# aubin-tchoi/shot-fpfh

Hardware: AMD Instinct MI355X
Metric: descriptors/sec (SHOT+FPFH) on 1M-pt cloud (higher is better)
Workload: dtype f64

## Files before the change

### shot_fpfh_amd/csrc/search.hip

```cpp
#include <algorithm>
#include <cmath>
#include <numeric>

#include "host_stage.h"
#include "search_util.h"

sf_grid_desc sf_make_grid_desc(const sf_cloud *c)
{
    sf_grid_desc g;
    for (int a = 0; a < 3; ++a) {
        g.lo[a] = c->lo[a];
        g.dim[a] = c->dim[a];
    }
    g.inv_cell = c->inv_cell;
    g.inv_cell_x = c->inv_cell * c->xsub;
    g.cell = c->cell;
    g.xsub = c->xsub;
    return g;
}

namespace {

__device__ unsigned long long sf_k2_paths[2];
template <int MODE, bool SEL, bool SHARE = false, bool DBG = false>
__global__ __launch_bounds__(64 * SF_K2_WPB) void k_radius(sf_grid_desc g, const int32_t *__restrict__ cell_start,
                                                const double *__restrict__ xs, const double *__restrict__ ys,
                                                const double *__restrict__ zs, const double *__restrict__ qx,
                                                const double *__restrict__ qy, const double *__restrict__ qz,
                                                int64_t m, double r2, int cap, int32_t *__restrict__ count,
                                                int64_t *__restrict__ offset, int32_t *__restrict__ idx,
                                                const int32_t *__restrict__ qsel)
{
    const int lane = threadIdx.x & 63, sl = lane & 15, rw = lane >> 4;
    const int64_t q0 = sf_uniform64((sf_xcd_block() * SF_K2_WPB + (threadIdx.x >> 6)) * 4);
    if (q0 >= m) return;
    const int nq = (int)(m - q0 < 4 ? m - q0 : 4);
    const int64_t qm0 = q0 + (rw < nq ? rw : 0);
    const int64_t qm = SEL ? (int64_t)qsel[qm0] : qm0;
    const double pxv = qx[qm], pyv = qy[qm], pzv = qz[qm];
    int y0, y1, z0, z1;
    stencil_bounds(pyv, g.lo[1], g.inv_cell, g.dim[1], y0, y1);
    stencil_bounds(pzv, g.lo[2], g.inv_cell, g.dim[2], z0, z1);
    __shared__ int4 runs[SF_K2_WPB][4][12];
    __shared__ int stages[MODE != 0 ? SF_K2_WPB : 1][SHARE ? 4 : 1][256];
    static_assert(!SHARE || (MODE == 2 && !SEL), "the shared sweep serves the single sweep into slots");
    int4(*const tabs)[12] = runs[threadIdx.x >> 6];
    bool share = false;
    int s, e;
    sf_k2_window(g, cell_start, pxv, pyv, pzv, r2, sl, rw < nq, y0, y1, z0, z1, s, e);
    if (SHARE) {
        const bool same = y0 == sf_uniform(y0) && y1 == sf_uniform(y1) && z0 == sf_uniform(z0) && z1 == sf_uniform(z1);
        share = nq == 4 && __ballot(same) == ~0ull;
        if (share) {
            int us = e > s ? s : 0x7fffffff, ue = e > s ? e : 0;
            us = min(us, __shfl_xor(us, 16));
            ue = max(ue, __shfl_xor(ue, 16));
            us = min(us, __shfl_xor(us, 32));
            ue = max(ue, __shfl_xor(ue, 32));
            s = ue ? us : 0;
            e = ue;
        }
    }
    const int first_slot = sf_k2_store_runs(s, e, sl, tabs[rw]);
    __builtin_amdgcn_wave_barrier();
    if (DBG && lane == 0) atomicAdd(&sf_k2_paths[share ? 0 : 1], 1ull);
    if (SHARE && share) {
        const int4 *const tab = tabs[0];
        const int b4 = __builtin_amdgcn_readlane(first_slot, 4), b8 = __builtin_amdgcn_readlane(first_slot, 8);
        const int nslots = __builtin_amdgcn_readlane(first_slot, 9);
        double px[4], py[4], pz[4];
        int total[4], flushed[4];
#pragma unroll
        for (int qi = 0; qi < 4; ++qi) {
            px[qi] = sf_read_lane(pxv, 16 * qi);
            py[qi] = sf_read_lane(pyv, 16 * qi);
            pz[qi] = sf_read_lane(pzv, 16 * qi);
            total[qi] = 0;
            flushed[qi] = 0;
        }
        int32_t *const out0 = idx + q0 * (int64_t)cap;
        for (int f0 = 0; f0 < nslots; f0 += 64) {
            const sf_k2_pair c = sf_k2_load_pair(tab, b4, b8, nslots, f0 + lane, xs, ys, zs);
            const int j = c.j;
            const unsigned long long i0 = __builtin_amdgcn_ballot_w64(c.in0), i1 = __builtin_amdgcn_ballot_w64(c.in1);
#pragma unroll
            for (int qi = 0; qi < 4; ++qi) {
                const double dxa = c.X.x - px[qi], dya = c.Y.x - py[qi], dza = c.Z.x - pz[qi];
                const double dxb = c.X.y - px[qi], dyb = c.Y.y - py[qi], dzb = c.Z.y - pz[qi];
                const double d2a = (dxa * dxa + dya * dya) + dza * dza, d2b = (dxb * dxb + dyb * dyb) + dzb * dzb;
                const bool hit0 = c.in0 & (d2a <= r2);
                const bool hit1 = c.in1 & (d2b <= r2);
                const unsigned long long m0 = __builtin_amdgcn_ballot_w64(d2a <= r2) & i0, m1 = __builtin_amdgcn_ballot_w64(d2b <= r2) & i1;
                int *const stage = stages[threadIdx.x >> 6][qi];
                const int2 pos = sf_k2_hit_pos(total[qi], m0, m1, hit0);
                if (hit0 && pos.x < cap) stage[pos.x & 255] = j;
                if (hit1 && pos.y < cap) stage[pos.y & 255] = j + 1;
                total[qi] += __popcll(m0) + __popcll(m1);
                const int have = total[qi] < cap ? total[qi] : cap;
                while (have - flushed[qi] >= 64) {
                    SF_LIST_STORE(out0 + qi * (int64_t)cap + flushed[qi] + lane, stage[(flushed[qi] + lane) & 255]);
                    flushed[qi] += 64;
                }
            }
        }
#pragma unroll
        for (int qi = 0; qi < 4; ++qi) {
            const int *const stage = stages[threadIdx.x >> 6][qi];
            const int have = total[qi] < cap ? total[qi] : cap;
            if (flushed[qi] + lane < have) SF_LIST_STORE(out0 + qi * (int64_t)cap + flushed[qi] + lane, stage[(flushed[qi] + lane) & 255]);
            if (lane == 0) {
                const int64_t q = q0 + qi;
                count[q] = total[qi];
                offset[q] = q * (int64_t)cap;
                if (q == m - 1) {
                    count[m] = 0;
                    offset[m] = (q + 1) * (int64_t)cap;
                }
            }
        }
        return;
    }
    for (int qi = 0; qi < nq; ++qi) {
        const int64_t q = SEL ? (int64_t)sf_uniform(__shfl((int)qm, 16 * qi)) : q0 + qi;
        const int4 *const tab = tabs[qi];
        const double px = __shfl(pxv, 16 * qi), py = __shfl(pyv, 16 * qi), pz = __shfl(pzv, 16 * qi);
        const int b4 = __shfl(first_slot, 16 * qi + 4), b8 = __shfl(first_slot, 16 * qi + 8);
#ifdef SF_K2_ABLATE
        const int nslots = sf_uniform(__shfl(first_slot, 16 * qi + 9)) * SF_K2_ABLATE / 100;
#else
        const int nslots = sf_uniform(__shfl(first_slot, 16 * qi + 9));
#endif
        int total = 0;
        const int64_t out = MODE == 1 ? offset[q] : q * (int64_t)cap;
        const int room = MODE == 2 ? cap : 0x7fffffff;
        int *const stage = stages[threadIdx.x >> 6][0];
        int flushed = 0;
        for (int f0 = 0; f0 < nslots; f0 += 64) {
            const sf_k2_pair c = sf_k2_load_pair(tab, b4, b8, nslots, f0 + lane, xs, ys, zs);
            const int j = c.j;
            const double dxa = c.X.x - px, dya = c.Y.x - py, dza = c.Z.x - pz;
            const double dxb = c.X.y - px, dyb = c.Y.y - py, dzb = c.Z.y - pz;
            const double d2a = (dxa * dxa + dya * dya) + dza * dza, d2b = (dxb * dxb + dyb * dyb) + dzb * dzb;
            const bool hit0 = c.in0 & (d2a <= r2);
            const bool hit1 = c.in1 & (d2b <= r2);
            const unsigned long long m0 = __ballot(hit0), m1 = __ballot(hit1);
            if (MODE != 0) {
                const int2 pos = sf_k2_hit_pos(total, m0, m1, hit0);
                if (hit0 && pos.x < room) stage[pos.x & 255] = j;
                if (hit1 && pos.y < room) stage[pos.y & 255] = j + 1;
            }
            total += __popcll(m0) + __popcll(m1);
            if (MODE != 0) {
                const int have = total < room ? total : room;
                while (have - flushed >= 64) {
                    SF_LIST_STORE(idx + out + flushed + lane, stage[(flushed + lane) & 255]);
                    flushed += 64;
                }
            }
        }
        if (MODE != 0) {
            const int have = total < room ? total : room;
            if (flushed + lane < have) SF_LIST_STORE(idx + out + flushed + lane, stage[(flushed + lane) & 255]);
        }
        if (lane == 0) {
            if (MODE != 1) {
                count[SEL ? q0 + qi : q] = total;
                if (!SEL && q == m - 1) count[m] = 0;
            }
            if (MODE == 2) {
                offset[q] = out;
                if (q == m - 1) offset[m] = out + cap;
            }
        }
    }
}

#ifndef SF_K2C_WPB
#define SF_K2C_WPB 4
#endif
#ifndef SF_K2C_LIST
#define SF_K2C_LIST 192
#endif
struct sf_cov_list { double x[SF_K2C_LIST], y[SF_K2C_LIST], z[SF_K2C_LIST]; };

__global__ __launch_bounds__(64 * SF_K2C_WPB) __attribute__((amdgpu_waves_per_eu(7))) void k_radius_cov(sf_grid_desc g, const int32_t *__restrict__ cell_start,
                                                const double *__restrict__ xs, const double *__restrict__ ys,
                                                const double *__restrict__ zs, const double *__restrict__ qx,
                                                const double *__restrict__ qy, const double *__restrict__ qz,
                                                int64_t m, double r2, double *__restrict__ cov, double *__restrict__ bary,
                                                int32_t *__restrict__ count)
{
    const int lane = threadIdx.x & 63, sl = lane & 15, rw = lane >> 4;
    const int64_t q0 = sf_uniform64((sf_xcd_block() * SF_K2C_WPB + (threadIdx.x >> 6)) * 4);
    if (q0 >= m) return;
    const int nq = (int)(m - q0 < 4 ? m - q0 : 4);
    const int64_t qm = q0 + (rw < nq ? rw : 0);
    const double pxv = qx[qm], pyv = qy[qm], pzv = qz[qm];
    int y0, y1, z0, z1;
    stencil_bounds(pyv, g.lo[1], g.inv_cell, g.dim[1], y0, y1);
    stencil_bounds(pzv, g.lo[2], g.inv_cell, g.dim[2], z0, z1);
    __shared__ int4 runs[SF_K2C_WPB][4][12];
    __shared__ sf_cov_list lists[SF_K2C_WPB];
    int4(*const tabs)[12] = runs[threadIdx.x >> 6];
    sf_cov_list &L = lists[threadIdx.x >> 6];
    int s, e;
    sf_k2_window(g, cell_start, pxv, pyv, pzv, r2, sl, rw < nq, y0, y1, z0, z1, s, e);
    const int first_slot = sf_k2_store_runs(s, e, sl, tabs[rw]);
    __builtin_amdgcn_wave_barrier();
#define SF_K2C_LDS_SYNC()                                                                                            \
    do {                                                                                                            \
        __builtin_amdgcn_fence(__ATOMIC_RELEASE, "wavefront");                                                      \
        __builtin_amdgcn_wave_barrier();                                                                            \
        __builtin_amdgcn_fence(__ATOMIC_ACQUIRE, "wavefront");                                                      \
    } while (0)
    for (int qi = 0; qi < nq; ++qi) {
        const int64_t q = q0 + qi;
        const int4 *const tab = tabs[qi];
        const double px = __shfl(pxv, 16 * qi), py = __shfl(pyv, 16 * qi), pz = __shfl(pzv, 16 * qi);
        const int b4 = __shfl(first_slot, 16 * qi + 4), b8 = __shfl(first_slot, 16 * qi + 8);
        const int nslots = sf_uniform(__shfl(first_slot, 16 * qi + 9));
        auto sweep = [&](int keep, bool wrap, auto &&after_step) -> int {
            int total = 0;
            for (int f0 = 0; f0 < nslots; f0 += 64) {
                const sf_k2_pair c = sf_k2_load_pair(tab, b4, b8, nslots, f0 + lane, xs, ys, zs);
                const double dxa = c.X.x - px, dya = c.Y.x - py, dza = c.Z.x - pz;
                const double dxb = c.X.y - px, dyb = c.Y.y - py, dzb = c.Z.y - pz;
                const double d2a = (dxa * dxa + dya * dya) + dza * dza, d2b = (dxb * dxb + dyb * dyb) + dzb * dzb;
                const bool hit0 = c.in0 & (d2a <= r2);
                const bool hit1 = c.in1 & (d2b <= r2);
                const unsigned long long m0 = __ballot(hit0), m1 = __ballot(hit1);
                const int2 pos = sf_k2_hit_pos(total, m0, m1, hit0);
                const int s0 = wrap ? pos.x % SF_K2C_LIST : pos.x, s1 = wrap ? pos.y % SF_K2C_LIST : pos.y;
                if (hit0 && pos.x < keep) { L.x[s0] = dxa; L.y[s0] = dya; L.z[s0] = dza; }
                if (hit1 && pos.y < keep) { L.x[s1] = dxb; L.y[s1] = dyb; L.z[s1] = dzb; }
                total += __popcll(m0) + __popcll(m1);
                after_step(total);
            }
            return total;
        };
        SF_K2C_LDS_SYNC();
        const int k = sweep(SF_K2C_LIST, false, [](int) {});
        SF_K2C_LDS_SYNC();
        const double kk = (double)k, ik = 1.0 / kk;
        double sx = 0.0, sy = 0.0, sz = 0.0;
        double part[8] = {0, 0, 0, 0, 0, 0, 0, 0};
        double mx, my, mz;
        if (k <= SF_K2C_LIST) {
            for (int t = lane; t < k; t += 64) { sx += L.x[t]; sy += L.y[t]; sz += L.z[t]; }
            {
                const double bs[4] = {sx, sy, sz, 0.0};
                const double bt = sf_wave_sum4(bs);
                mx = sf_read_lane(bt, 0) * ik; my = sf_read_lane(bt, 16) * ik; mz = sf_read_lane(bt, 32) * ik;
            }
            for (int t = lane; t < k; t += 64) {
                const double ax = L.x[t] - mx, ay = L.y[t] - my, az = L.z[t] - mz;
                part[0] += ax * ax;
                part[1] += ay * ax;
                part[2] += az * ax;
                part[3] += ay * ay;
                part[4] += az * ay;
                part[5] += az * az;
            }
        } else {
            int done = 0;
            auto bary_step = [&](int total) {
                if (done + 64 <= total) {
                    SF_K2C_LDS_SYNC();
                    while (done + 64 <= total) {
                        const int t = (done + lane) % SF_K2C_LIST;
                        sx += L.x[t]; sy += L.y[t]; sz += L.z[t];
                        done += 64;
                    }
                    SF_K2C_LDS_SYNC();
                }
            };
            sweep(0x7fffffff, true, bary_step);
            SF_K2C_LDS_SYNC();
            if (done + lane < k) { const int t = (done + lane) % SF_K2C_LIST; sx += L.x[t]; sy += L.y[t]; sz += L.z[t]; }
            {
                const double bs[4] = {sx, sy, sz, 0.0};
                const double bt = sf_wave_sum4(bs);
                mx = sf_read_lane(bt, 0) * ik; my = sf_read_lane(bt, 16) * ik; mz = sf_read_lane(bt, 32) * ik;
            }
            auto add_moments = [&](int t) {
                const double ax = L.x[t] - mx, ay = L.y[t] - my, az = L.z[t] - mz;
                part[0] += ax * ax;
                part[1] += ay * ax;
                part[2] += az * ax;
                part[3] += ay * ay;
                part[4] += az * ay;
                part[5] += az * az;
            };
            done = 0;
            auto mom_step = [&](int total) {
                if (done + 64 <= total) {
                    SF_K2C_LDS_SYNC();
                    while (done + 64 <= total) {
                        add_moments((done + lane) % SF_K2C_LIST);
                        done += 64;
                    }
                    SF_K2C_LDS_SYNC();
                }
            };
            SF_K2C_LDS_SYNC();
            sweep(0x7fffffff, true, mom_step);
            SF_K2C_LDS_SYNC();
            if (done + lane < k) add_moments((done + lane) % SF_K2C_LIST);
        }
        const double tot = sf_wave_sum8(part);
        const int e = lane >> 3;
        if ((lane & 7) == 0 && e < 6) cov[6 * q + e] = tot * ik;
        if (bary && lane == 0) { bary[3 * q] = mx; bary[3 * q + 1] = my; bary[3 * q + 2] = mz; }
        if (count && lane == 0) count[q] = k;
    }
#undef SF_K2C_LDS_SYNC
}

__global__ void k_query_cells(const double *__restrict__ q, int64_t m, sf_grid_desc g, int32_t *__restrict__ cid,
                              int32_t *__restrict__ val)
{
    int64_t i = (int64_t)blockIdx.x * blockDim.x + threadIdx.x;
    if (i >= m) return;
    int cx = sf_cell_coord(q[3 * i + 0], g.lo[0], g.inv_cell_x, g.dim[0]);
    int cy = sf_cell_coord(q[3 * i + 1], g.lo[1], g.inv_cell, g.dim[1]);
    int cz = sf_cell_coord(q[3 * i + 2], g.lo[2], g.inv_cell, g.dim[2]);
    cid[i] = (cz * g.dim[1] + cy) * g.dim[0] + cx;
    val[i] = (int32_t)i;
// ... 187 lines not shown
    }
    nb->planned = true;
    nb->main_chunks = chunks;
    nb->n_mid = 0;
    for (int c = chunks; c < 4; ++c) nb->n_mid += nb->hist[c];
    if (chunks == need) nb->n_mid = 0;
    nb->tail_limit = 255;
    nb->n_tail = nb->hist[4];
    if (nb->max_count <= nb->tail_limit) { nb->tail_limit = 0x7fffffff; nb->n_tail = 0; }
    if (nb->n_mid) SF_CHECK(select_slots(ctx, m, count_between{nb->count, 64 * chunks, 255}, nb->n_mid, &nb->mid_sel));
    if (nb->n_tail) SF_CHECK(select_longer(ctx, nb->count, m, nb->tail_limit, nb->n_tail, &nb->tail_sel));
    return SF_OK;
}

static int64_t capacity_from(const sf_cloud *c, double mean, int64_t mx)
{
    int64_t v = (int64_t)(std::max(mean * 2.25, 1.15 * (double)mx)) + 32;
    return std::min<int64_t>(((v + 31) / 32) * 32, std::max<int64_t>(((c->n + 31) / 32) * 32, 32));
}

static int sample_capacity(sf_ctx *ctx, sf_cloud *c, sf_nbrs *nb, const sf_grid_desc &g, double r2, int64_t *cap)
{
    const int64_t m = nb->m, stride = m / SF_K2_SAMPLE;
    sf_pool_guard tmp(ctx);
    int32_t *sel = nullptr, *cnt = nullptr;
    void *pin = nullptr;
    SF_CHECK(tmp.alloc(&sel, (size_t)SF_K2_SAMPLE));
    SF_CHECK(tmp.alloc(&cnt, (size_t)SF_K2_SAMPLE));
    SF_CHECK(sf_ctx_pinned(ctx, &pin));
    static_assert(SF_K2_SAMPLE * sizeof(int32_t) <= SF_PINNED_BYTES, "sample exceeds the pinned words");
    SF_LAUNCH(ctx, "k2_sample", k_iota_stride, dim3(SF_K2_SAMPLE / 256), dim3(256), sel, (int64_t)SF_K2_SAMPLE, stride);
    SF_LAUNCH(ctx, "k2_sample", (k_radius<0, true>), dim3(sf_xcd_grid(sf_div_up(SF_K2_SAMPLE, 4 * SF_K2_WPB))), dim3(64 * SF_K2_WPB), g,
              c->cell_start, c->xs, c->ys, c->zs, nb->qx, nb->qy, nb->qz, (int64_t)SF_K2_SAMPLE, r2, 0, cnt, (int64_t *)nullptr,
              (int32_t *)nullptr, (const int32_t *)sel);
    SF_HIP(hipMemcpyAsync(pin, cnt, SF_K2_SAMPLE * sizeof(int32_t), hipMemcpyDeviceToHost, ctx->stream));
    SF_HIP(hipStreamSynchronize(ctx->stream));
    const int32_t *h = (const int32_t *)pin;
    double sum = 0.0;
    int32_t mx = 0;
    for (int i = 0; i < SF_K2_SAMPLE; ++i) { sum += h[i]; mx = std::max(mx, h[i]); }
    *cap = capacity_from(c, sum / SF_K2_SAMPLE, mx);
    return SF_OK;
}

int sf_k2_count_sample(sf_ctx *ctx, sf_cloud *c, sf_nbrs *nb, double r2, int32_t *sel_dev, int32_t *cnt_dev)
{
    const sf_grid_desc g = sf_make_grid_desc(c);
    sf_launch_timer t_(ctx, "k2_sample");
    hipLaunchKernelGGL(k_iota_stride, dim3(SF_K2_SAMPLE / 256), dim3(256), 0, ctx->stream, sel_dev, (int64_t)SF_K2_SAMPLE, nb->m / SF_K2_SAMPLE);
    hipLaunchKernelGGL((k_radius<0, true>), dim3(sf_xcd_grid(sf_div_up(SF_K2_SAMPLE, 4 * SF_K2_WPB))), dim3(64 * SF_K2_WPB), 0, ctx->stream, g,
                       c->cell_start, c->xs, c->ys, c->zs, nb->qx, nb->qy, nb->qz, (int64_t)SF_K2_SAMPLE, r2, 0, cnt_dev, (int64_t *)nullptr,
                       (int32_t *)nullptr, (const int32_t *)sel_dev);
    SF_HIP(hipGetLastError());
    return SF_OK;
}

static int exact_scan_fill(sf_ctx *ctx, sf_cloud *c, sf_nbrs *nb, const sf_grid_desc &g, const dim3 &grid, const dim3 &block, double r2)
{
    const int64_t m = nb->m;
    {
        sf_pool_guard tmp(ctx);
        auto in = rocprim::make_transform_iterator(nb->count, to_i64());
        SF_CHECK(sf_rocprim(ctx, tmp, "k2_scan", true, [&](void *t, size_t &tb) {
            return rocprim::exclusive_scan(t, tb, in, nb->offset, (int64_t)0, (size_t)(m + 1), rocprim::plus<int64_t>(), ctx->stream);
        }));
    }
    SF_CHECK(sf_palloc(ctx, &nb->idx, (size_t)nb->total + 4));
    nb->cap = 0;
    if (nb->total) {
        SF_LAUNCH(ctx, "k2_radius_fill", (k_radius<1, false>), grid, block, g, c->cell_start, c->xs, c->ys, c->zs, nb->qx, nb->qy,
                  nb->qz, m, r2, 0, nb->count, nb->offset, nb->idx, (const int32_t *)nullptr);
    }
    return SF_OK;
}

static int run_search(sf_ctx *ctx, sf_cloud *c, sf_nbrs *nb)
{
    const int64_t m = nb->m;
    const double r2 = nb->radius * nb->radius;
    SF_CHECK(sf_palloc(ctx, &nb->count, (size_t)(m + 1)));
    SF_CHECK(sf_palloc(ctx, &nb->offset, (size_t)(m + 1)));
    if (!m) {
        SF_HIP(hipMemsetAsync(nb->count, 0, sizeof(int32_t), ctx->stream));
        SF_HIP(hipMemsetAsync(nb->offset, 0, sizeof(int64_t), ctx->stream));
    }
    sf_grid_desc g = sf_make_grid_desc(c);
    const dim3 grid(sf_xcd_grid(sf_div_up(m ? m : 1, 4 * SF_K2_WPB))), block(64 * SF_K2_WPB);
    if (!m) {
        if (ctx->collective_stats && ctx->comm) {
            const sf_cloud::search_key ekey{nb->radius, c->cell, c->xsub, nb->self_begin, 0};
            const bool seen = nb->self && !getenv("SF_K2_NO_HINT") && c->search_records.count(ekey);
            if (!seen || getenv("SF_K2_CHECK_RECORD")) {
                SF_CHECK(count_stats(ctx, nb, 0x7fffffff, nullptr));
                if (nb->self) {
                    sf_cloud::search_record r;
                    r.max_count_all = (int32_t)nb->max_count_all;
                    r.folded = true;
                    c->search_records[ekey] = r;
                }
            } else {
                nb->max_count_all = c->search_records[ekey].max_count_all;
            }
        }
        SF_CHECK(sf_palloc(ctx, &nb->idx, (size_t)8));
        return SF_OK;
    }
    int64_t cap = 0;
    bool optimistic = m >= 8 * SF_K2_SAMPLE && !getenv("SF_K2_EXACT");
    if (optimistic) {
        auto hint = c->list_stats.find({nb->radius, nb->self});
        if (hint != c->list_stats.end() && !getenv("SF_K2_NO_HINT")) cap = capacity_from(c, hint->second.first, hint->second.second);
        else SF_CHECK(sample_capacity(ctx, c, nb, g, r2, &cap));
        if (const char *e = getenv("SF_K2_CAP")) { const long v = atol(e); if (v >= 32) cap = (v / 32) * 32; }
        const int64_t most = std::max<int64_t>(((((int64_t)24 << 30) / (4 * m)) / 32) * 32, 32);
        if (cap > most) cap = std::max<int64_t>(most, 64);
        optimistic = cap * m * 4 <= ((int64_t)24 << 30) && cap < 0x7fffffff;
    }
    if (!optimistic) {
        SF_LAUNCH(ctx, "k2_radius_count", (k_radius<0, false>), grid, block, g, c->cell_start, c->xs, c->ys, c->zs, nb->qx, nb->qy,
                  nb->qz, m, r2, 0, nb->count, nb->offset, (int32_t *)nullptr, (const int32_t *)nullptr);
        const sf_cloud::search_key xkey{nb->radius, c->cell, c->xsub, nb->self_begin, -m};
        auto xit = nb->self && !getenv("SF_K2_NO_HINT") && !getenv("SF_K2_CHECK_RECORD") ? c->search_records.find(xkey) : c->search_records.end();
        if (xit != c->search_records.end() && (xit->second.folded || !(ctx->collective_stats && ctx->comm))) {
            const sf_cloud::search_record &r = xit->second;
            nb->total = r.total;
            nb->max_count = r.max_count;
            nb->max_count_all = r.max_count_all;
            nb->n_overflow = 0;
            for (int h = 0; h < 5; ++h) nb->hist[h] = r.hist[h];
        } else {
            SF_CHECK(count_stats(ctx, nb, 0x7fffffff, nullptr));
            if (nb->self) {
                if (c->search_records.size() > 256) c->search_records.clear();
                sf_cloud::search_record r;
                r.total = nb->total; r.max_count = nb->max_count; r.max_count_all = nb->max_count_all;
                for (int h = 0; h < 5; ++h) r.hist[h] = nb->hist[h];
                r.folded = ctx->collective_stats && ctx->comm;
                c->search_records[xkey] = r;
            }
        }
        SF_CHECK(exact_scan_fill(ctx, c, nb, g, grid, block, r2));
        return plan_dispatch(ctx, c, nb);
    }
    const sf_cloud::search_key rkey{nb->radius, c->cell, c->xsub, nb->self_begin, m};
    const sf_cloud::search_record *rec = nullptr;
    if (nb->self && !getenv("SF_K2_NO_HINT")) {
        auto it = c->search_records.find(rkey);
        if (it != c->search_records.end() && (it->second.folded || !(ctx->collective_stats && ctx->comm))) rec = &it->second;
    }
    if (rec) cap = rec->cap;
    SF_CHECK(sf_palloc(ctx, &nb->idx, (size_t)(cap * m) + 4));
    nb->cap = cap;
    const char *const sh = getenv("SF_K2_SHARED");
    const int shared = sh ? atoi(sh) : 1;
    auto *const k_slots = shared == 2 ? k_radius<2, false, true, true> : shared ? k_radius<2, false, true> : k_radius<2, false>;
    SF_LAUNCH(ctx, "k2_radius_slots", k_slots, grid, block, g, c->cell_start, c->xs, c->ys, c->zs, nb->qx, nb->qy,
              nb->qz, m, r2, (int)cap, nb->count, nb->offset, nb->idx, (const int32_t *)nullptr);
    int64_t ovf_total = 0;
    if (rec && !getenv("SF_K2_CHECK_RECORD")) {
        nb->total = rec->total;
        nb->max_count = rec->max_count;
        nb->max_count_all = rec->max_count_all;
        nb->n_overflow = rec->n_overflow;
        for (int h = 0; h < 5; ++h) nb->hist[h] = rec->hist[h];
        ovf_total = rec->ovf_total;
    } else {
        SF_CHECK(count_stats(ctx, nb, (int)cap, &ovf_total));
        if (rec && (nb->total != rec->total || nb->max_count != rec->max_count || nb->n_overflow != rec->n_overflow ||
                    ovf_total != rec->ovf_total || nb->hist[4] != rec->hist[4] || nb->hist[0] != rec->hist[0])) {
            sf_set_error("sf_radius_search_self: the lists of positions %lld .. + %lld at radius %g differ from the record of the previous "
                         "search of that range (total %lld / %lld)", (long long)nb->self_begin, (long long)m, nb->radius,
                         (long long)nb->total, (long long)rec->total);
            return SF_ERR_STATE;
        }
        if (nb->self) {
            if (c->search_records.size() > 256) c->search_records.clear();
            sf_cloud::search_record r;
            r.total = nb->total; r.n_overflow = nb->n_overflow; r.ovf_total = ovf_total; r.cap = cap;
            for (int h = 0; h < 5; ++h) r.hist[h] = nb->hist[h];
            r.max_count = nb->max_count; r.max_count_all = nb->max_count_all;
            r.folded = ctx->collective_stats && ctx->comm;
            if (r.n_overflow) {
                const int64_t most = std::max<int64_t>(((((int64_t)24 << 30) / (4 * m)) / 32) * 32, 32);
                const int64_t cap2 = capacity_from(c, (double)nb->total / (double)m, nb->max_count);
                if (cap2 >= nb->max_count && cap2 <= most) { r.cap = cap2; r.n_overflow = 0; r.ovf_total = 0; }
            }
            c->search_records[rkey] = r;
        }
    }
    if (nb->n_overflow * 2 > m) {
        sf_pool_release(ctx, nb->idx);
        nb->idx = nullptr;
        nb->n_overflow = 0;
        SF_CHECK(exact_scan_fill(ctx, c, nb, g, grid, block, r2));
        return plan_dispatch(ctx, c, nb);
    }
    if (nb->n_overflow) {
        const int64_t no = nb->n_overflow;
        sf_pool_guard tmp(ctx);
        int32_t *sel = nullptr;
        int64_t *off = nullptr;
        SF_CHECK(select_longer(ctx, nb->count, m, (int)cap, no, &sel));
        tmp.held.push_back(sel);
        SF_CHECK(tmp.alloc(&off, (size_t)no));
        auto in = rocprim::make_transform_iterator((const int32_t *)sel, count_of{nb->count});
        SF_CHECK(sf_rocprim(ctx, tmp, "k2_scan", true, [&](void *t, size_t &tb) {
            return rocprim::exclusive_scan(t, tb, in, off, (int64_t)0, (size_t)no, rocprim::plus<int64_t>(), ctx->stream);
        }));
        SF_CHECK(sf_palloc(ctx, &nb->idx_ovf, (size_t)ovf_total + 4));
        const int64_t delta = (int64_t)(((intptr_t)nb->idx_ovf - (intptr_t)nb->idx) / (intptr_t)sizeof(int32_t));
        SF_LAUNCH(ctx, "k2_select", k_patch_offsets, dim3((unsigned)sf_div_up(no, 256)), dim3(256), (const int32_t *)sel,
                  (const int64_t *)off, no, delta, nb->offset);
        SF_LAUNCH(ctx, "k2_radius_refill", (k_radius<1, true>), dim3(sf_xcd_grid(sf_div_up(no, 4 * SF_K2_WPB))), block, g, c->cell_start,
                  c->xs, c->ys, c->zs, nb->qx, nb->qy, nb->qz, no, r2, 0, nb->count, nb->offset, nb->idx, (const int32_t *)sel);
    }
    return plan_dispatch(ctx, c, nb);
}

static int ensure_grid(sf_ctx *ctx, sf_cloud *c, double radius, int64_t need_begin = 0, int64_t need_end = -1)
{
    if (!(radius > 0.0) || !std::isfinite(radius)) {
        sf_set_error("radius must be positive and finite (got %g)", radius);
        return SF_ERR_ARG;
    }
    const bool covers = need_end < 0 ? (c->pop_begin == 0 && c->pop_end == c->n)
                                     : (need_begin >= c->pop_begin && need_end <= c->pop_end);
    if (c->cell_start && covers && c->cell >= radius && c->cell <= 2.0 * radius * (1.0 + 1e-6)) return SF_OK;
    return sf_cloud_build_grid(ctx, c, radius);
}

extern "C" sf_nbrs *sf_radius_search_self(sf_ctx *ctx, sf_cloud *c, double radius, int64_t begin, int64_t end)
{
    if (!ctx || !c) { sf_set_error("sf_radius_search_self: null argument"); return nullptr; }
    if (begin < 0 || end > c->n || begin > end) {
        sf_set_error("sf_radius_search_self: bad range [%lld, %lld) for n=%lld", (long long)begin, (long long)end,
                     (long long)c->n);
        return nullptr;
    }
    if (hipSetDevice(ctx->device) != hipSuccess) { sf_set_error("hipSetDevice failed"); return nullptr; }
    if (ensure_grid(ctx, c, radius, begin, end) != SF_OK) return nullptr;
    sf_nbrs *nb = new sf_nbrs();
    nb->m = end - begin;
    nb->radius = radius;
    nb->self = true;
    nb->self_begin = begin;
    nb->qx = c->xs + begin;
    nb->qy = c->ys + begin;
    nb->qz = c->zs + begin;
    sf_nbrs_stamp(nb, c);
    if (run_search(ctx, c, nb) != SF_OK) {
        sf_nbrs_free(ctx, nb);
        return nullptr;
    }
    return nb;
}

int sf_k2_prepare_queries(sf_ctx *ctx, sf_cloud *c, sf_nbrs *nb, const double *queries, int flags)
{
    const int64_t m = nb->m;
    size_t mm = (size_t)(m ? m : 1);
    double *dq = nullptr;
    bool own_dq = false;
    if (flags & SF_IN_DEVICE) {
        dq = const_cast<double *>(queries);
    } else {
        SF_CHECK(sf_palloc(ctx, &dq, mm * 3));
        own_dq = true;
        if (m) SF_HIP(hipMemcpyAsync(dq, queries, (size_t)m * 24, hipMemcpyHostToDevice, ctx->stream));
    }
    SF_CHECK(sf_palloc(ctx, &nb->qx, mm));
    SF_CHECK(sf_palloc(ctx, &nb->qy, mm));
    SF_CHECK(sf_palloc(ctx, &nb->qz, mm));
    SF_CHECK(sf_palloc(ctx, &nb->qrow, mm));
    if (m) {
        sf_pool_guard tmp(ctx);
        int32_t *cid = nullptr, *cid_s = nullptr, *val = nullptr;
        SF_CHECK(tmp.alloc(&cid, mm));
        SF_CHECK(tmp.alloc(&cid_s, mm));
        SF_CHECK(tmp.alloc(&val, mm));
        sf_grid_desc g = sf_make_grid_desc(c);
        SF_LAUNCH(ctx, "k2_query_cells", k_query_cells, dim3((unsigned)sf_div_up(m, 256)), dim3(256), dq, m, g, cid,
                  val);
        int bits = 1;
        while (((int64_t)1 << bits) < c->ncell) ++bits;
        SF_CHECK(sf_rocprim(ctx, tmp, "k2_query_sort", true, [&](void *t, size_t &tb) {
            return rocprim::radix_sort_pairs<sf_sort_config>(t, tb, cid, cid_s, val, nb->qrow, (size_t)m, 0, bits, ctx->stream);
        }));
        SF_LAUNCH(ctx, "k2_gather_queries", k_gather_queries, dim3((unsigned)sf_div_up(m, 256)), dim3(256), dq,
                  nb->qrow, m, nb->qx, nb->qy, nb->qz);
    }
    if (own_dq) {
        SF_HIP(hipStreamSynchronize(ctx->stream));
        sf_pool_release(ctx, dq);
    }
    return SF_OK;
}

extern "C" sf_nbrs *sf_radius_search(sf_ctx *ctx, sf_cloud *c, const double *queries, int64_t m, double radius,
                                     int flags)
{
    if (!ctx || !c || (!queries && m > 0) || m < 0 || m > 2147483000LL) {
        sf_set_error("sf_radius_search: bad arguments (m=%lld)", (long long)m);
        return nullptr;
    }
    if (hipSetDevice(ctx->device) != hipSuccess) { sf_set_error("hipSetDevice failed"); return nullptr; }
    if (ensure_grid(ctx, c, radius) != SF_OK) return nullptr;
    sf_nbrs *nb = new sf_nbrs();
    nb->m = m;
    nb->radius = radius;
    nb->self = false;
// ... 362 lines not shown
```

### shot_fpfh_amd/csrc/search_util.h

```cpp
#pragma once
#include "common.h"
#include "dev_prims.h"
#include "device_util.h"

namespace {


struct to_i64 {
    __host__ __device__ int64_t operator()(int32_t v) const { return (int64_t)v; }
};

__device__ inline void stencil_bounds(double v, double lo, double inv_cell, int dim, int &c0, int &c1)
{
    double t = floor((v - lo) * inv_cell);
    double top = (double)(dim - 1);
    double a = t - 1.0, b = t + 1.0;
    if (!(a >= 0.0)) a = 0.0;
    if (a > top) a = top;
    if (!(b >= 0.0)) b = 0.0;
    if (b > top) b = top;
    c0 = (int)a;
    c1 = (int)b;
}


#ifndef SF_K2_WPB
#define SF_K2_WPB 8
#endif

__device__ __forceinline__ void sf_k2_window(const sf_grid_desc &g, const int32_t *__restrict__ cell_start, double px, double py,
                                             double pz, double r2, int sl, bool row_live, int y0, int y1, int z0, int z1, int &s,
                                             int &e)
{
    const int r = sl < 9 ? sl : 8;
    const int cz = z0 + r / 3, cy = y0 + r % 3;
    bool ok = sl < 9 && row_live && cz <= z1 && cy <= y1;
    const int64_t row = ((int64_t)(ok ? cz : z0) * g.dim[1] + (ok ? cy : y0)) * g.dim[0];
    const double pxr = px - g.lo[0], pyr = py - g.lo[1], pzr = pz - g.lo[2];
    const double by0 = (double)cy * g.cell, bz0 = (double)cz * g.cell;
    const double slack_y = 1e-9 * g.cell + 1e-15 * (fabs(pyr) + by0 + g.cell);
    const double slack_z = 1e-9 * g.cell + 1e-15 * (fabs(pzr) + bz0 + g.cell);
    const double dy = fmax(fmax(by0 - pyr, pyr - (by0 + g.cell)) - slack_y, 0.0);
    const double dz = fmax(fmax(bz0 - pzr, pzr - (bz0 + g.cell)) - slack_z, 0.0);
    const double w2 = (r2 * (1.0 + 1e-9) - dy * dy) - dz * dz;
    ok = ok && w2 >= 0.0;
    const double w = sf_sqrt_fast(fmax(w2, 0.0)) * (1.0 + 1e-9) + 1e-9 * g.cell +
                     1e-15 * (fabs(pxr) + (double)g.dim[0] * (g.cell / (double)g.xsub));
    s = 0;
    e = 0;
    if (sl < 9) {
        s = cell_start[row + sf_cell_coord(pxr - w, 0.0, g.inv_cell_x, g.dim[0])];
        e = cell_start[row + sf_cell_coord(pxr + w, 0.0, g.inv_cell_x, g.dim[0]) + 1];
    }
    if (!ok) { s = 0; e = 0; }
}

__device__ __forceinline__ int sf_k2_store_runs(int s, int e, int sl, int4 *tab_row)
{
    const int base = s & ~1;
    const int npairs = (e - base + 1) >> 1;
    int inc = npairs;
    inc += __builtin_amdgcn_update_dpp(0, inc, 0x111, 0xf, 0xf, false);
    inc += __builtin_amdgcn_update_dpp(0, inc, 0x112, 0xf, 0xf, false);
    inc += __builtin_amdgcn_update_dpp(0, inc, 0x114, 0xf, 0xf, false);
    inc += __builtin_amdgcn_update_dpp(0, inc, 0x118, 0xf, 0xf, false);
    const int first_slot = inc - npairs;
    if (sl < 12) tab_row[sl] = make_int4(base - 2 * first_slot, s, e, first_slot);
    return first_slot;
}

struct sf_k2_pair {
    int j;
    bool in0, in1;
    double2 X, Y, Z;
};
__device__ __forceinline__ sf_k2_pair sf_k2_load_pair(const int4 *tab, int b4, int b8, int nslots, int f, const double *__restrict__ xs,
                                                      const double *__restrict__ ys, const double *__restrict__ zs)
{
    int r = f >= b4 ? 4 : 0;
    r += f >= tab[r + 2].w ? 2 : 0;
    r += f >= tab[r + 1].w ? 1 : 0;
    r = f >= b8 ? 8 : r;
    const int4 t = tab[r];
    const bool live = f < nslots;
    sf_k2_pair p;
    p.j = live ? t.x + 2 * f : 0;
    p.in0 = live & (p.j >= t.y);
    p.in1 = live & (p.j + 1 < t.z);
    p.X = *reinterpret_cast<const double2 *>(xs + p.j);
    p.Y = *reinterpret_cast<const double2 *>(ys + p.j);
    p.Z = *reinterpret_cast<const double2 *>(zs + p.j);
    return p;
}

__device__ __forceinline__ int2 sf_k2_hit_pos(int total, unsigned long long m0, unsigned long long m1, bool hit0)
{
    const int pos = total + sf_prefix_count(m0) + sf_prefix_count(m1);
    return make_int2(pos, pos + (hit0 ? 1 : 0));
}

#define SF_K2_SAMPLE 2048

struct sf_identity {
    template <typename T> __host__ __device__ T operator()(T v) const { return v; }
};
template <typename S, typename T, typename F>
__global__ void k_perm_scatter(const S *__restrict__ sorted, const int32_t *__restrict__ perm, int64_t n, T *__restrict__ out, F f)
{
    const int64_t i = (int64_t)blockIdx.x * blockDim.x + threadIdx.x;
    if (i < n) out[perm[i]] = f(sorted[i]);
}
template <typename T>
__global__ void k_perm_gather(const T *__restrict__ src, const int32_t *__restrict__ perm, int64_t n, int pad, T *__restrict__ sorted)
{
    const int64_t i = (int64_t)blockIdx.x * blockDim.x + threadIdx.x;
    if (i < n) sorted[i] = src[perm[i]];
    else if (i < n + pad) sorted[i] = T(0);
}
template <typename S, typename T, typename F = sf_identity>
int sf_perm_scatter(sf_ctx *ctx, const char *name, const sf_cloud *c, const S *sorted, T *out, F f = F())
{
    SF_LAUNCH(ctx, name, (k_perm_scatter<S, T, F>), dim3((unsigned)sf_div_up(c->n, 256)), dim3(256), sorted, (const int32_t *)c->perm, c->n, out, f);
    return SF_OK;
}
template <typename T>
int sf_perm_gather(sf_ctx *ctx, const char *name, const sf_cloud *c, const T *src, int pad, T *sorted)
{
    SF_LAUNCH(ctx, name, k_perm_gather<T>, dim3((unsigned)sf_div_up(c->n + pad, 256)), dim3(256), src, (const int32_t *)c->perm, c->n, pad, sorted);
    return SF_OK;
}

}

int sf_k2_prepare_queries(sf_ctx *ctx, sf_cloud *c, sf_nbrs *nb, const double *queries, int flags);
int sf_k2_count_sample(sf_ctx *ctx, sf_cloud *c, sf_nbrs *nb, double r2, int32_t *sel_dev, int32_t *cnt_dev);
int sf_k2_ensure_grid(sf_ctx *ctx, sf_cloud *c, double radius);
int sf_k2_own_grid(sf_ctx *ctx, sf_cloud *c, double radius);
int sf_k2_radius_cov_self(sf_ctx *ctx, sf_cloud *c, double radius, const char *prof, double *cov, int32_t *count);
int sf_k2_count_self(sf_ctx *ctx, sf_cloud *c, double radius, const char *prof, int32_t *count);
int sf_k2_ball_sizes(sf_ctx *ctx, sf_cloud *c, sf_pool_guard &g, double radius, const char *prof, int32_t **count);
```

Baseline: 611.6 million.

## Share candidate sweep across eight queries per wave in radius search

Adds a new radius-search kernel in which each wave handles eight queries instead of four. When all eight share the same y/z stencil, it builds a single union candidate window and tests every loaded candidate pair against all eight query points read from LDS. This amortizes candidate loads and the window and run-table setup over more queries. It also uses a 128-entry ring per query with spill handling, and a single-point tail that handles leftover slots at half-pair granularity. The new kernel is the default; in exchange it uses more LDS per block, adds per-hit bookkeeping, and scans a wider union window when the eight queries' x ranges differ.

```diff
diff --git a/shot_fpfh_amd/csrc/search.hip b/shot_fpfh_amd/csrc/search.hip
--- a/shot_fpfh_amd/csrc/search.hip
+++ b/shot_fpfh_amd/csrc/search.hip
@@ -22,18 +22,17 @@
 namespace {
 
 __device__ unsigned long long sf_k2_paths[2];
-template <int MODE, bool SEL, bool SHARE = false, bool DBG = false>
-__global__ __launch_bounds__(64 * SF_K2_WPB) void k_radius(sf_grid_desc g, const int32_t *__restrict__ cell_start,
-                                                const double *__restrict__ xs, const double *__restrict__ ys,
-                                                const double *__restrict__ zs, const double *__restrict__ qx,
-                                                const double *__restrict__ qy, const double *__restrict__ qz,
-                                                int64_t m, double r2, int cap, int32_t *__restrict__ count,
-                                                int64_t *__restrict__ offset, int32_t *__restrict__ idx,
-                                                const int32_t *__restrict__ qsel)
+template <int MODE, bool SEL, bool SHARE, bool DBG, bool QLDS = false>
+__device__ __forceinline__ void sf_k2_four(const sf_grid_desc &g, const int32_t *__restrict__ cell_start,
+                                           const double *__restrict__ xs, const double *__restrict__ ys,
+                                           const double *__restrict__ zs, const double *__restrict__ qx,
+                                           const double *__restrict__ qy, const double *__restrict__ qz,
+                                           int64_t m, double r2, int cap, int32_t *__restrict__ count,
+                                           int64_t *__restrict__ offset, int32_t *__restrict__ idx,
+                                           const int32_t *__restrict__ qsel, const int64_t q0, int4 (*const tabs)[12],
+                                           int (*const stages)[256], double *const qc = nullptr)
 {
     const int lane = threadIdx.x & 63, sl = lane & 15, rw = lane >> 4;
-    const int64_t q0 = sf_uniform64((sf_xcd_block() * SF_K2_WPB + (threadIdx.x >> 6)) * 4);
-    if (q0 >= m) return;
     const int nq = (int)(m - q0 < 4 ? m - q0 : 4);
     const int64_t qm0 = q0 + (rw < nq ? rw : 0);
     const int64_t qm = SEL ? (int64_t)qsel[qm0] : qm0;
@@ -41,10 +40,7 @@
     int y0, y1, z0, z1;
     stencil_bounds(pyv, g.lo[1], g.inv_cell, g.dim[1], y0, y1);
     stencil_bounds(pzv, g.lo[2], g.inv_cell, g.dim[2], z0, z1);
-    __shared__ int4 runs[SF_K2_WPB][4][12];
-    __shared__ int stages[MODE != 0 ? SF_K2_WPB : 1][SHARE ? 4 : 1][256];
     static_assert(!SHARE || (MODE == 2 && !SEL), "the shared sweep serves the single sweep into slots");
-    int4(*const tabs)[12] = runs[threadIdx.x >> 6];
     bool share = false;
     int s, e;
     sf_k2_window(g, cell_start, pxv, pyv, pzv, r2, sl, rw < nq, y0, y1, z0, z1, s, e);
@@ -70,11 +66,15 @@
         const int nslots = __builtin_amdgcn_readlane(first_slot, 9);
         double px[4], py[4], pz[4];
         int total[4], flushed[4];
+        if (QLDS) {
+            if (sl == 0) { qc[rw] = pxv; qc[8 + rw] = pyv; qc[16 + rw] = pzv; }
+            __builtin_amdgcn_wave_barrier();
+        }
 #pragma unroll
         for (int qi = 0; qi < 4; ++qi) {
-            px[qi] = sf_read_lane(pxv, 16 * qi);
-            py[qi] = sf_read_lane(pyv, 16 * qi);
-            pz[qi] = sf_read_lane(pzv, 16 * qi);
+            px[qi] = QLDS ? 0.0 : sf_read_lane(pxv, 16 * qi);
+            py[qi] = QLDS ? 0.0 : sf_read_lane(pyv, 16 * qi);
+            pz[qi] = QLDS ? 0.0 : sf_read_lane(pzv, 16 * qi);
             total[qi] = 0;
             flushed[qi] = 0;
         }
@@ -83,15 +83,18 @@
             const sf_k2_pair c = sf_k2_load_pair(tab, b4, b8, nslots, f0 + lane, xs, ys, zs);
             const int j = c.j;
             const unsigned long long i0 = __builtin_amdgcn_ballot_w64(c.in0), i1 = __builtin_amdgcn_ballot_w64(c.in1);
+            int step0 = 0;
+            if (QLDS) asm volatile("" : "+v"(step0));
 #pragma unroll
             for (int qi = 0; qi < 4; ++qi) {
-                const double dxa = c.X.x - px[qi], dya = c.Y.x - py[qi], dza = c.Z.x - pz[qi];
-                const double dxb = c.X.y - px[qi], dyb = c.Y.y - py[qi], dzb = c.Z.y - pz[qi];
+                const double qpx = QLDS ? qc[step0 + qi] : px[qi], qpy = QLDS ? qc[step0 + 8 + qi] : py[qi], qpz = QLDS ? qc[step0 + 16 + qi] : pz[qi];
+                const double dxa = c.X.x - qpx, dya = c.Y.x - qpy, dza = c.Z.x - qpz;
+                const double dxb = c.X.y - qpx, dyb = c.Y.y - qpy, dzb = c.Z.y - qpz;
                 const double d2a = (dxa * dxa + dya * dya) + dza * dza, d2b = (dxb * dxb + dyb * dyb) + dzb * dzb;
                 const bool hit0 = c.in0 & (d2a <= r2);
                 const bool hit1 = c.in1 & (d2b <= r2);
                 const unsigned long long m0 = __builtin_amdgcn_ballot_w64(d2a <= r2) & i0, m1 = __builtin_amdgcn_ballot_w64(d2b <= r2) & i1;
-                int *const stage = stages[threadIdx.x >> 6][qi];
+                int *const stage = stages[qi];
                 const int2 pos = sf_k2_hit_pos(total[qi], m0, m1, hit0);
                 if (hit0 && pos.x < cap) stage[pos.x & 255] = j;
                 if (hit1 && pos.y < cap) stage[pos.y & 255] = j + 1;
@@ -105,7 +108,7 @@
         }
 #pragma unroll
         for (int qi = 0; qi < 4; ++qi) {
-            const int *const stage = stages[threadIdx.x >> 6][qi];
+            const int *const stage = stages[qi];
             const int have = total[qi] < cap ? total[qi] : cap;
             if (flushed[qi] + lane < have) SF_LIST_STORE(out0 + qi * (int64_t)cap + flushed[qi] + lane, stage[(flushed[qi] + lane) & 255]);
             if (lane == 0) {
@@ -133,7 +136,7 @@
         int total = 0;
         const int64_t out = MODE == 1 ? offset[q] : q * (int64_t)cap;
         const int room = MODE == 2 ? cap : 0x7fffffff;
-        int *const stage = stages[threadIdx.x >> 6][0];
+        int *const stage = stages[0];
         int flushed = 0;
         for (int f0 = 0; f0 < nslots; f0 += 64) {
             const sf_k2_pair c = sf_k2_load_pair(tab, b4, b8, nslots, f0 + lane, xs, ys, zs);
@@ -173,6 +176,163 @@
             }
         }
     }
+}
+
+template <int MODE, bool SEL, bool SHARE = false, bool DBG = false>
+__global__ __launch_bounds__(64 * SF_K2_WPB) void k_radius(sf_grid_desc g, const int32_t *__restrict__ cell_start,
+                                                const double *__restrict__ xs, const double *__restrict__ ys,
+                                                const double *__restrict__ zs, const double *__restrict__ qx,
+                                                const double *__restrict__ qy, const double *__restrict__ qz,
+                                                int64_t m, double r2, int cap, int32_t *__restrict__ count,
+                                                int64_t *__restrict__ offset, int32_t *__restrict__ idx,
+                                                const int32_t *__restrict__ qsel)
+{
+    const int64_t q0 = sf_uniform64((sf_xcd_block() * SF_K2_WPB + (threadIdx.x >> 6)) * 4);
+    if (q0 >= m) return;
+    __shared__ int4 runs[SF_K2_WPB][4][12];
+    __shared__ int stages[MODE != 0 ? SF_K2_WPB : 1][SHARE ? 4 : 1][256];
+    sf_k2_four<MODE, SEL, SHARE, DBG>(g, cell_start, xs, ys, zs, qx, qy, qz, m, r2, cap, count, offset, idx, qsel, q0,
+                                      runs[threadIdx.x >> 6], stages[MODE != 0 ? threadIdx.x >> 6 : 0]);
+}
+
+#ifndef SF_K2_WPB8
+#define SF_K2_WPB8 8
+#endif
+#define SF_K2_RING8 128
+template <bool DBG>
+__global__ __launch_bounds__(64 * SF_K2_WPB8) __attribute__((amdgpu_waves_per_eu(6))) void k_radius8(sf_grid_desc g, const int32_t *__restrict__ cell_start,
+                                                const double *__restrict__ xs, const double *__restrict__ ys,
+                                                const double *__restrict__ zs, const double *__restrict__ qx,
+                                                const double *__restrict__ qy, const double *__restrict__ qz,
+                                                int64_t m, double r2, int cap, int32_t *__restrict__ count,
+                                                int64_t *__restrict__ offset, int32_t *__restrict__ idx)
+{
+    const int lane = threadIdx.x & 63, sl = lane & 15, rw = lane >> 4, wv = threadIdx.x >> 6;
+    const int64_t q0 = sf_uniform64((sf_xcd_block() * SF_K2_WPB8 + wv) * 8);
+    if (q0 >= m) return;
+    __shared__ int4 runs[SF_K2_WPB8][4][12];
+    __shared__ double qcs[SF_K2_WPB8][3][8];
+    __shared__ int stages[SF_K2_WPB8][8 * SF_K2_RING8];
+    static_assert(8 * SF_K2_RING8 == 4 * 256, "the two halves' four-query sweeps run in the same LDS");
+    int4(*const tabs)[12] = runs[wv];
+    if (m - q0 >= 8) {
+        const double pxa = qx[q0 + rw], pya = qy[q0 + rw], pza = qz[q0 + rw];
+        const double pxb = qx[q0 + rw + 4], pyb = qy[q0 + rw + 4], pzb = qz[q0 + rw + 4];
+        int y0, y1, z0, z1, yb0, yb1, zb0, zb1;
+        stencil_bounds(pya, g.lo[1], g.inv_cell, g.dim[1], y0, y1);
+        stencil_bounds(pza, g.lo[2], g.inv_cell, g.dim[2], z0, z1);
+        stencil_bounds(pyb, g.lo[1], g.inv_cell, g.dim[1], yb0, yb1);
+        stencil_bounds(pzb, g.lo[2], g.inv_cell, g.dim[2], zb0, zb1);
+        const int uy0 = sf_uniform(y0), uy1 = sf_uniform(y1), uz0 = sf_uniform(z0), uz1 = sf_uniform(z1);
+        const bool same = (y0 == uy0) & (y1 == uy1) & (z0 == uz0) & (z1 == uz1) & (yb0 == uy0) & (yb1 == uy1) & (zb0 == uz0) & (zb1 == uz1);
+        if (__ballot(same) == ~0ull) {
+            int s, e;
+            sf_k2_window2(g, cell_start, pxa, pya, pza, pxb, pyb, pzb, r2, sl, y0, y1, z0, z1, s, e);
+            int us = e > s ? s : 0x7fffffff, ue = e > s ? e : 0;
+            us = min(us, __shfl_xor(us, 16));
+            ue = max(ue, __shfl_xor(ue, 16));
+            us = min(us, __shfl_xor(us, 32));
+            ue = max(ue, __shfl_xor(ue, 32));
+            s = ue ? us : 0;
+            e = ue;
+            const int first_slot = sf_k2_store_runs(s, e, sl, tabs[rw]);
+            if (sl == 0) {
+                qcs[wv][0][rw] = pxa; qcs[wv][1][rw] = pya; qcs[wv][2][rw] = pza;
+                qcs[wv][0][rw + 4] = pxb; qcs[wv][1][rw + 4] = pyb; qcs[wv][2][rw + 4] = pzb;
+            }
+            __builtin_amdgcn_wave_barrier();
+            if (DBG && lane == 0) atomicAdd(&sf_k2_paths[0], 1ull);
+            const int4 *const tab = tabs[0];
+            const int b4 = __builtin_amdgcn_readlane(first_slot, 4), b8 = __builtin_amdgcn_readlane(first_slot, 8);
+            const int nslots = __builtin_amdgcn_readlane(first_slot, 9);
+            const double *const cq = qcs[wv][0];
+            int total[8], flushed[8];
+#pragma unroll
+            for (int qi = 0; qi < 8; ++qi) {
+                total[qi] = 0;
+                flushed[qi] = 0;
+            }
+            int32_t *const out0 = idx + q0 * (int64_t)cap;
+            int f0 = 0;
+            for (; nslots - f0 > 32; f0 += 64) {
+                const sf_k2_pair c = sf_k2_load_pair(tab, b4, b8, nslots, f0 + lane, xs, ys, zs);
+                const int j = c.j;
+                const unsigned long long i0 = __builtin_amdgcn_ballot_w64(c.in0), i1 = __builtin_amdgcn_ballot_w64(c.in1);
+                int step0 = 0;
+                asm volatile("" : "+v"(step0));
+                double nx = cq[step0], ny = cq[step0 + 8], nz = cq[step0 + 16];
+#pragma unroll
+                for (int qi = 0; qi < 8; ++qi) {
+                    const double px = nx, py = ny, pz = nz;
+                    if (qi < 7) { nx = cq[step0 + qi + 1]; ny = cq[step0 + qi + 9]; nz = cq[step0 + qi + 17]; }
+                    const double dxa = c.X.x - px, dya = c.Y.x - py, dza = c.Z.x - pz;
+                    const double dxb = c.X.y - px, dyb = c.Y.y - py, dzb = c.Z.y - pz;
+                    const double d2a = (dxa * dxa + dya * dya) + dza * dza, d2b = (dxb * dxb + dyb * dyb) + dzb * dzb;
+                    const bool hit0 = c.in0 & (d2a <= r2);
+                    const bool hit1 = c.in1 & (d2b <= r2);
+                    const unsigned long long m0 = __builtin_amdgcn_ballot_w64(d2a <= r2) & i0, m1 = __builtin_amdgcn_ballot_w64(d2b <= r2) & i1;
+                    int *const stage = stages[wv] + SF_K2_RING8 * qi;
+                    const int2 pos = sf_k2_hit_pos(total[qi], m0, m1, hit0);
+                    int lim = flushed[qi] + SF_K2_RING8;
+                    const int room = lim < cap ? lim : cap;
+                    if (hit0 && pos.x < room) stage[pos.x & (SF_K2_RING8 - 1)] = j;
+                    if (hit1 && pos.y < room) stage[pos.y & (SF_K2_RING8 - 1)] = j + 1;
+                    total[qi] += __popcll(m0) + __popcll(m1);
+                    const int have = total[qi] < cap ? total[qi] : cap;
+                    while (have - flushed[qi] >= 64) {
+                        SF_LIST_STORE(out0 + qi * (int64_t)cap + flushed[qi] + lane, stage[(flushed[qi] + lane) & (SF_K2_RING8 - 1)]);
+                        flushed[qi] += 64;
+                        if (have > lim) {
+                            const int room2 = have < lim + 64 ? have : lim + 64;
+                            if (hit0 && pos.x >= lim && pos.x < room2) stage[pos.x & (SF_K2_RING8 - 1)] = j;
+                            if (hit1 && pos.y >= lim && pos.y < room2) stage[pos.y & (SF_K2_RING8 - 1)] = j + 1;
+                            lim += 64;
+                        }
+                    }
+                }
+            }
+            if (f0 < nslots) {
+                const sf_k2_single c = sf_k2_load_single(tab, b4, b8, nslots, f0, lane, xs, ys, zs);
+                const unsigned long long in = __builtin_amdgcn_ballot_w64(c.in);
+#pragma unroll
+                for (int qi = 0; qi < 8; ++qi) {
+                    const double px = cq[qi], py = cq[qi + 8], pz = cq[qi + 16];
+                    const double dx = c.x - px, dy = c.y - py, dz = c.z - pz;
+                    const double d2 = (dx * dx + dy * dy) + dz * dz;
+                    const bool hit = c.in & (d2 <= r2);
+                    const unsigned long long mh = __builtin_amdgcn_ballot_w64(d2 <= r2) & in;
+                    int *const stage = stages[wv] + SF_K2_RING8 * qi;
+                    const int pos = total[qi] + sf_prefix_count(mh);
+                    if (hit && pos < cap) stage[pos & (SF_K2_RING8 - 1)] = c.j;
+                    total[qi] += __popcll(mh);
+                    const int have = total[qi] < cap ? total[qi] : cap;
+                    if (have - flushed[qi] >= 64) {
+                        SF_LIST_STORE(out0 + qi * (int64_t)cap + flushed[qi] + lane, stage[(flushed[qi] + lane) & (SF_K2_RING8 - 1)]);
+                        flushed[qi] += 64;
+                    }
+                }
+            }
+#pragma unroll
+            for (int qi = 0; qi < 8; ++qi) {
+                const int *const stage = stages[wv] + SF_K2_RING8 * qi;
+                const int have = total[qi] < cap ? total[qi] : cap;
+                if (flushed[qi] + lane < have) SF_LIST_STORE(out0 + qi * (int64_t)cap + flushed[qi] + lane, stage[(flushed[qi] + lane) & (SF_K2_RING8 - 1)]);
+                if (lane == 0) {
+                    const int64_t q = q0 + qi;
+                    count[q] = total[qi];
+                    offset[q] = q * (int64_t)cap;
+                    if (q == m - 1) {
+                        count[m] = 0;
+                        offset[m] = (q + 1) * (int64_t)cap;
+                    }
+                }
+            }
+            return;
+        }
+    }
+    if (DBG && lane == 0) atomicAdd(&sf_k2_paths[1], 1ull);
+    sf_k2_four<2, false, true, false, true>(g, cell_start, xs, ys, zs, qx, qy, qz, m, r2, cap, count, offset, idx, (const int32_t *)nullptr, q0, tabs, (int(*)[256])stages[wv], qcs[wv][0]);
+    if (q0 + 4 < m) sf_k2_four<2, false, true, false, true>(g, cell_start, xs, ys, zs, qx, qy, qz, m, r2, cap, count, offset, idx, (const int32_t *)nullptr, q0 + 4, tabs, (int(*)[256])stages[wv], qcs[wv][0]);
 }
 
 #ifndef SF_K2C_WPB
@@ -666,10 +826,17 @@
     SF_CHECK(sf_palloc(ctx, &nb->idx, (size_t)(cap * m) + 4));
     nb->cap = cap;
     const char *const sh = getenv("SF_K2_SHARED");
-    const int shared = sh ? atoi(sh) : 1;
-    auto *const k_slots = shared == 2 ? k_radius<2, false, true, true> : shared ? k_radius<2, false, true> : k_radius<2, false>;
-    SF_LAUNCH(ctx, "k2_radius_slots", k_slots, grid, block, g, c->cell_start, c->xs, c->ys, c->zs, nb->qx, nb->qy,
-              nb->qz, m, r2, (int)cap, nb->count, nb->offset, nb->idx, (const int32_t *)nullptr);
+    const int shared = sh ? atoi(sh) : 8;
+    if (shared == 8 || shared == 3) {
+        const dim3 grid8(sf_xcd_grid(sf_div_up(m, 8 * SF_K2_WPB8))), block8(64 * SF_K2_WPB8);
+        auto *const k_slots8 = shared == 3 ? k_radius8<true> : k_radius8<false>;
+        SF_LAUNCH(ctx, "k2_radius_slots", k_slots8, grid8, block8, g, c->cell_start, c->xs, c->ys, c->zs, nb->qx, nb->qy,
+                  nb->qz, m, r2, (int)cap, nb->count, nb->offset, nb->idx);
+    } else {
+        auto *const k_slots = shared == 2 ? k_radius<2, false, true, true> : shared ? k_radius<2, false, true> : k_radius<2, false>;
+        SF_LAUNCH(ctx, "k2_radius_slots", k_slots, grid, block, g, c->cell_start, c->xs, c->ys, c->zs, nb->qx, nb->qy,
+                  nb->qz, m, r2, (int)cap, nb->count, nb->offset, nb->idx, (const int32_t *)nullptr);
+    }
     int64_t ovf_total = 0;
     if (rec && !getenv("SF_K2_CHECK_RECORD")) {
         nb->total = rec->total;
diff --git a/shot_fpfh_amd/csrc/search_util.h b/shot_fpfh_amd/csrc/search_util.h
--- a/shot_fpfh_amd/csrc/search_util.h
+++ b/shot_fpfh_amd/csrc/search_util.h
@@ -55,6 +55,43 @@
     if (!ok) { s = 0; e = 0; }
 }
 
+__device__ __forceinline__ void sf_k2_window2(const sf_grid_desc &g, const int32_t *__restrict__ cell_start, double pxa, double pya,
+                                              double pza, double pxb, double pyb, double pzb, double r2, int sl, int y0, int y1,
+                                              int z0, int z1, int &s, int &e)
+{
+    const int r = sl < 9 ? sl : 8;
+    const int cz = z0 + r / 3, cy = y0 + r % 3;
+    const bool in_stencil = sl < 9 && cz <= z1 && cy <= y1;
+    const int64_t row = ((int64_t)(in_stencil ? cz : z0) * g.dim[1] + (in_stencil ? cy : y0)) * g.dim[0];
+    const double by0 = (double)cy * g.cell, bz0 = (double)cz * g.cell;
+    const double xext = (double)g.dim[0] * (g.cell / (double)g.xsub);
+    double lo = 1.0e300, hi = -1.0e300;
+    bool any = false;
+    auto reach = [&](double px, double py, double pz) {
+        const double pxr = px - g.lo[0], pyr = py - g.lo[1], pzr = pz - g.lo[2];
+        const double slack_y = 1e-9 * g.cell + 1e-15 * (fabs(pyr) + by0 + g.cell);
+        const double slack_z = 1e-9 * g.cell + 1e-15 * (fabs(pzr) + bz0 + g.cell);
+        const double dy = fmax(fmax(by0 - pyr, pyr - (by0 + g.cell)) - slack_y, 0.0);
+        const double dz = fmax(fmax(bz0 - pzr, pzr - (bz0 + g.cell)) - slack_z, 0.0);
+        const double w2 = (r2 * (1.0 + 1e-9) - dy * dy) - dz * dz;
+        const double w = sf_sqrt_fast(fmax(w2, 0.0)) * (1.0 + 1e-9) + 1e-9 * g.cell + 1e-15 * (fabs(pxr) + xext);
+        if (w2 >= 0.0) {
+            lo = fmin(lo, pxr - w);
+            hi = fmax(hi, pxr + w);
+            any = true;
+        }
+    };
+    reach(pxa, pya, pza);
+    reach(pxb, pyb, pzb);
+    s = 0;
+    e = 0;
+    if (sl < 9) {
+        s = cell_start[row + sf_cell_coord(lo, 0.0, g.inv_cell_x, g.dim[0])];
+        e = cell_start[row + sf_cell_coord(hi, 0.0, g.inv_cell_x, g.dim[0]) + 1];
+    }
+    if (!(in_stencil && any)) { s = 0; e = 0; }
+}
+
 __device__ __forceinline__ int sf_k2_store_runs(int s, int e, int sl, int4 *tab_row)
 {
     const int base = s & ~1;
@@ -93,6 +130,31 @@
     return p;
 }
 
+struct sf_k2_single {
+    int j;
+    bool in;
+    double x, y, z;
+};
+__device__ __forceinline__ sf_k2_single sf_k2_load_single(const int4 *tab, int b4, int b8, int nslots, int f0, int lane,
+                                                          const double *__restrict__ xs, const double *__restrict__ ys,
+                                                          const double *__restrict__ zs)
+{
+    const int f = f0 + (lane >> 1);
+    int r = f >= b4 ? 4 : 0;
+    r += f >= tab[r + 2].w ? 2 : 0;
+    r += f >= tab[r + 1].w ? 1 : 0;
+    r = f >= b8 ? 8 : r;
+    const int4 t = tab[r];
+    const bool live = f < nslots;
+    sf_k2_single p;
+    p.j = live ? t.x + 2 * f + (lane & 1) : 0;
+    p.in = live & (p.j >= t.y) & (p.j < t.z);
+    p.x = xs[p.j];
+    p.y = ys[p.j];
+    p.z = zs[p.j];
+    return p;
+}
+
 __device__ __forceinline__ int2 sf_k2_hit_pos(int total, unsigned long long m0, unsigned long long m1, bool hit0)
 {
     const int pos = total + sf_prefix_count(m0) + sf_prefix_count(m1);
```

Result: no change. 610.1 million (-0.2%).
